# wjqkkky/TTS

Measured on AMD Instinct MI355X. Metric: mel-frames/s (Tacotron2-DDC + MB-MelGAN end-to-end), higher is better.
Workload: dtype f32; 1 GPU; C2: Tacotron2-DDC (r_init=7, r=2, sigmoid attn) + MB-MelGAN [8,4,2]x4, 32 LJ-length utterances per GPU; global_batch=32, r=2, parallelism=replicas x1

## Files before the change

tts_amd/_lib.py:

```python

import atexit
import collections
import ctypes
import os
import threading
from typing import Dict

import numpy as np

_HERE = os.path.dirname(os.path.abspath(__file__))
LIB_PATH = os.environ.get("TTSHIP_LIB", os.path.join(_HERE, "libttship.so"))

_lib = None
_lock = threading.Lock()

_c_int_p = ctypes.POINTER(ctypes.c_int32)
_c_i64_p = ctypes.POINTER(ctypes.c_int64)
_c_f_p = ctypes.POINTER(ctypes.c_float)
_c_i_p = ctypes.POINTER(ctypes.c_int)
_vp = ctypes.c_void_p

SIGNATURES = [
    ("tts_version", ctypes.c_int, []),
    ("tts_last_error", ctypes.c_char_p, []),
# ... 449 lines not shown
    def pqmf_analysis(self, x, lens, H, y):
        B, L = x.shape
        l_a, l_p = _i32(lens)
        _check(self.lib.tts_pqmf_analysis(self.h, _ptr(x), l_p, B, L, H.shape[0], _ptr(H), H.shape[1] - 1, _ptr(y),
                                          y.shape[2], _stream(x.device)))

    def stft_pair_sums(self, y_hat, y, nsamples, n_fft, win_length, hop_length, sums):
        B, L = y.shape
        n_a, n_p = _i32(nsamples)
        _check(self.lib.tts_stft_pair_sums(self.h, _ptr(y_hat), _ptr(y), n_p, B, L, int(n_fft), int(win_length),
                                           int(hop_length), _ptr(sums), _stream(y.device)))

    def torch_stft_mag(self, wav, nsamples, n_fft, win_length, hop_length, mag):
        B, L = wav.shape
        n_a, n_p = _i32(nsamples)
        _check(self.lib.tts_torch_stft_mag(self.h, _ptr(wav), n_p, B, L, int(n_fft), int(win_length),
                                           int(hop_length), _ptr(mag), mag.shape[2], _stream(wav.device)))

    def conv_test(self, weight, bias, lens, src, out, max_q, device, transposed=False, K=1, dil=1, nphase=1,
                  pad_left=(0,), merged_u=0, src2=None, resid=None, resid_rows=0, aux=None, auxb=0, len_add=0,
                  in_mul=1, q_mul=1, out_mul=1, rep_pad=0, pad_mode=0, epi=0):
        w = np.ascontiguousarray(weight, dtype=np.float32)
        b = np.ascontiguousarray(bias, dtype=np.float32)
        lens_a = np.ascontiguousarray(lens, dtype=np.int32)
        d = ConvTest()
        d.h_weight, d.h_bias, d.h_lens = w.ctypes.data, b.ctypes.data, lens_a.ctypes.data
        d.transposed = int(bool(transposed))
        if transposed:
            d.Cin, d.Cout = w.shape[0], w.shape[1]
        else:
            d.Cout, d.Cin = w.shape[-3], w.shape[-2]
        assert len(b) == d.Cout
        d.K, d.dil, d.nphase, d.merged_u = K, dil, nphase, merged_u
        for i, p in enumerate(pad_left):
            d.pad_left[i] = p
        d.nsrc = 1 if src2 is None else 2
        for i, s in enumerate((src,) if src2 is None else (src, src2)):
            d.d_src[i] = s[0]
            for j in range(3):
                d.src_strides[i][j] = s[1][j]
            d.src_C[i], d.src_act[i] = s[2], s[3]
        d.d_out = out[0]
        for j in range(3):
            d.out_strides[j] = out[1][j]
        if resid is not None:
            d.d_resid = resid[0]
            for j in range(3):
                d.resid_strides[j] = resid[1][j]
        d.resid_rows, d.d_aux, d.auxb = resid_rows, aux, auxb
        d.B, d.max_q, d.len_add, d.in_mul, d.q_mul, d.out_mul = len(lens_a), max_q, len_add, in_mul, q_mul, out_mul
        d.rep_pad, d.pad_mode, d.epi = rep_pad, pad_mode, epi
        with self.lock:
            _check(self.lib.tts_test_conv(self.h, ctypes.c_void_p(ctypes.addressof(d)), _stream(device)))
        return bool(d.ran_x3), int(d.tq), int(d.range_flag)

    def decoder_stats(self):
        path, n = ctypes.c_int(0), ctypes.c_int(0)
        ms = (ctypes.c_float * 4)()
        st = (ctypes.c_int * 4)()
        _check(self.lib.tts_decoder_stats(self.h, ctypes.byref(path), ctypes.byref(n), ms, st))
        return int(path.value), [(float(ms[i]), int(st[i])) for i in range(n.value)]

    def set_gemm_mode(self, mode: str):
        if mode not in ("x3", "f32"):
            raise ValueError("gemm mode must be 'x3' or 'f32'")
        with self.lock:
            _check(self.lib.tts_set_gemm_mode(self.h, 1 if mode == "x3" else 0))

    def gemm_mode(self):
        m, n = ctypes.c_int(0), ctypes.c_int64(0)
        _check(self.lib.tts_gemm_mode(self.h, ctypes.byref(m), ctypes.byref(n)))
        return ("x3" if m.value else "f32"), int(n.value)

    def time_decoder_kernel(self, which: int, iters: int) -> float:
        ms = ctypes.c_float(0.0)
        _check(self.lib.tts_time_decoder_kernel(self.h, which, iters, ctypes.byref(ms)))
        return float(ms.value)


_engines: Dict[int, Engine] = {}


def get_engine(device) -> Engine:
    import torch
    dev = torch.device(device)
    if dev.type != "cuda":
        raise RuntimeError("tts_amd runs on MI355X (ROCm 'cuda' devices) only; got device "
                           f"'{dev}'. There is no CPU fallback: move the model with .cuda().")
    idx = dev.index if dev.index is not None else torch.cuda.current_device()
    with _lock:
        eng = _engines.get(idx)
    if eng is None:
        eng = Engine(idx)
        with _lock:
            _engines[idx] = eng
    return eng


@atexit.register
def _close_engines():
    with _lock:
        engines = list(_engines.values())
        _engines.clear()
    for eng in engines:
        try:
            eng.close()
# ... 3 lines not shown
```

tts_amd/csrc/api_core.hip:

```cpp
#include "host.h"
#include "split16.h"
#include "switches.h"

#include <cmath>
#include <cstring>
#include <memory>

static thread_local std::string g_err;
void tts_set_error(const std::string& m) { g_err = m; }

namespace ttsh {

__global__ void put_rows_kernel(int* dst, RowInts r, int n) {
  if ((int)threadIdx.x < n) dst[threadIdx.x] = r.v[threadIdx.x];
}

const int* put_rows(int* dst, const int32_t* h, int n, hipStream_t s) {
  for (int o = 0; o < n; o += BMAX) {
    const int m = std::min(BMAX, n - o);
    put_rows_kernel<<<1, BMAX, 0, s>>>(dst + o, row_ints(h + o, m), m);
    HIP_OK(hipGetLastError());
  }
  return dst;
}
// ... 147 lines not shown
  for (float v : Wm) wm_in_range &= std::fabs(v) < F16_RANGE;
  if (wm_in_range && conv_x3_supported(Cin, u * Cout, 2, 1)) {
    std::vector<float> bm((size_t)u * Cout);
    for (size_t r = 0; r < bm.size(); ++r) bm[r] = bias[r / u];
    pack_conv_x3_only(Lm, merge_convT_phases(Wm, u, Cin, Cout), bm, Cin, u * Cout, 2);
  } else {
    Lm.W16.reset();
  }
}

ConvRan run_conv(const ConvLayer& L, const ConvCall& c, hipStream_t st) {
  ConvArgs a{};
  a.src[0] = c.s[0];
  a.src[1] = c.nsrc > 1 ? c.s[1] : c.s[0];
  if (c.nsrc == 1) a.src[0].C = L.Cin;
  a.nsrc = c.nsrc;
  a.Cin = L.Cin;
  a.K = L.K;
  a.dil = L.dil;
  a.pad_mode = c.pad_mode;
  a.lens = c.lens;
  a.len_add = c.len_add;
  a.in_mul = c.in_mul;
  a.q_mul = c.q_mul;
  a.rep_pad = c.rep_pad;
  a.nphase = L.nphase;
  for (int i = 0; i < 8; ++i) a.pad_left[i] = L.pad_left[i];
  a.w_phase_stride = L.phase_stride;
  a.W = L.W.f();
  a.bias = L.bias.f();
  a.Cout = L.Cout;
  a.Cout_pad = L.Cout_pad;
  a.out = c.out;
  a.ob = c.ob;
  a.oc = c.oc;
  a.ot = c.ot;
  a.out_mul = c.out_mul;
  a.epi_act = c.epi;
  a.resid = c.resid;
  a.rb = c.rb;
  a.rc = c.rc;
  a.rt = c.rt;
  a.resid_rows = c.resid_rows;
  a.aux = c.aux;
  a.auxb = c.auxb;
  a.max_q = c.max_q;
  a.B = c.B;
  a.merged_u = c.merged_u;
  TTS_CHECK(!c.merged_u || (c.oflow && L.W16.p), "phase-merged ConvTranspose runs on split-f16 weights only");
  if (c.oflow && L.W16.p && c.nsrc == 1 && (c.s[0].sc != 1 || c.s[0].st % 4 == 0)) {
    a.W16 = L.W16.p;
    a.w16_phase_stride = L.w16_stride;
    a.oflow = c.oflow;
    return {true, launch_conv_x3(a, st)};
  }
  return {false, launch_conv(a, L.tile, st)};
}

void enter(tts_ctx* c, void* stream, bool join_voc) {
  if (c->sv_live && join_voc) {
    HIP_OK(hipStreamWaitEvent(c->s, c->ev_sv, 0));
    c->sv_live = false;
  }
  if (hipStreamQuery((hipStream_t)stream) == hipSuccess) return;
  (void)hipGetLastError();
  HIP_OK(hipEventRecord(c->ev_in, (hipStream_t)stream));
  HIP_OK(hipStreamWaitEvent(c->s, c->ev_in, 0));
}
void leave(tts_ctx* c, void* stream) {
  HIP_OK(hipEventRecord(c->ev_out, c->s));
  HIP_OK(hipStreamWaitEvent((hipStream_t)stream, c->ev_out, 0));
}

std::vector<float> lstm_tile_rows(const std::vector<float>& W, int H, int K) {
  std::vector<float> out((size_t)4 * H * K);
  for (int t = 0; t < H / 4; ++t)
    for (int g = 0; g < 4; ++g)
      for (int u = 0; u < 4; ++u) {
        const size_t src = (size_t)(g * H + 4 * t + u) * K, dst = (size_t)(t * 16 + g * 4 + u) * K;
        std::memcpy(&out[dst], &W[src], K * sizeof(float));
      }
  return out;
}

std::vector<float> hcat(const std::vector<std::pair<const float*, int>>& parts, int rows) {
  int K = 0;
  for (auto& p : parts) K += p.second;
  std::vector<float> out((size_t)rows * K);
  for (int r = 0; r < rows; ++r) {
    int off = 0;
    for (auto& p : parts) {
      std::memcpy(&out[(size_t)r * K + off], p.first + (size_t)r * p.second, p.second * sizeof(float));
      off += p.second;
    }
  }
  return out;
}

std::vector<float> slice_cols(const std::vector<float>& W, int rows, int K, int c0, int c1) {
  std::vector<float> out((size_t)rows * (c1 - c0));
  for (int r = 0; r < rows; ++r)
    std::memcpy(&out[(size_t)r * (c1 - c0)], &W[(size_t)r * K + c0], (c1 - c0) * sizeof(float));
  return out;
}

std::vector<float> swz(const std::vector<float>& Wm, int rows, int K) {
// ... 103 lines not shown
int tts_test_conv(tts_ctx* c, tts_conv_test* d, void* stream) {
  return guarded_ctx(c, [&] {
    TTS_CHECK(d && d->h_weight && d->h_bias && d->h_lens && d->d_src[0] && d->d_out, "test_conv: null argument");
    TTS_CHECK(d->Cin >= 1 && d->Cout >= 1 && d->B >= 1 && d->max_q >= 0, "test_conv: sizes");
    TTS_CHECK(d->nsrc == 1 || (d->nsrc == 2 && d->d_src[1] && d->src_C[0] + d->src_C[1] == d->Cin), "test_conv: sources");
    TTS_CHECK(d->nphase >= 1 && d->nphase <= 8, "conv: nphase");
    auto lay = [](const int64_t* s) {
      TTS_CHECK(s[1] >= 0 && s[2] >= 0 && s[1] < (1L << 31) && s[2] < (1L << 31), "test_conv: strides");
      return Layout{(long)s[0], (int)s[1], (int)s[2]};
    };
    d->ran_x3 = d->tq = 0;
    d->range_flag = 0;
    DeviceGuard g(c->device);
    enter(c, stream);
    ConvLayer L, Lm;
    const std::vector<float> bias(d->h_bias, d->h_bias + d->Cout);
    if (d->transposed) {
      const int u = d->nphase;
      TTS_CHECK(d->merged_u == 0 || d->merged_u == u, "test_conv: merged_u is 0 or the stride");
      pack_convT(L, Lm, std::vector<float>(d->h_weight, d->h_weight + (size_t)d->Cin * d->Cout * 2 * u), bias, u,
                 d->Cin, d->Cout);
    } else {
      TTS_CHECK(d->K >= 1 && d->dil >= 1 && d->merged_u == 0, "test_conv: taps");
      const size_t n = (size_t)d->nphase * d->Cout * d->Cin * d->K;
      pack_conv(L, std::vector<float>(d->h_weight, d->h_weight + n), bias, d->Cin, d->Cout, d->K, d->dil, d->nphase,
                d->pad_left);
    }
    DevBuf lens;
    ConvCall cc = conv_call(c, put_rows(lens, d->h_lens, d->B, c->s), d->B, d->max_q);
    cc.in(d->d_src[0], lay(d->src_strides[0]), d->nsrc == 2 ? d->src_C[0] : d->Cin, d->src_act[0]);
    if (d->nsrc == 2) {
      cc.in2(d->d_src[1], lay(d->src_strides[1]), d->src_C[1]);
      cc.s[1].act = d->src_act[1];
    }
    cc.to(d->d_out, lay(d->out_strides));
    if (d->d_resid) cc.add(d->d_resid, lay(d->resid_strides));
    cc.resid_rows = d->resid_rows;
    cc.aux = d->d_aux;
    cc.auxb = (long)d->auxb;
    cc.pad_mode = d->pad_mode;
    cc.len_add = d->len_add;
    cc.in_mul = d->in_mul;
    cc.q_mul = d->q_mul;
    cc.out_mul = d->out_mul;
    cc.rep_pad = d->rep_pad;
    cc.epi = d->epi;
    cc.merged_u = d->merged_u;
    if (cc.oflow) HIP_OK(hipMemsetAsync(cc.oflow, 0, 4, c->s));
    struct Sync {
      hipStream_t s;
      ~Sync() { (void)hipStreamSynchronize(s); }
    } sync{c->s};
    const ConvRan ran = run_conv(d->merged_u ? Lm : L, cc, c->s);
    d->ran_x3 = ran.x3 ? 1 : 0;
    d->tq = ran.tq;
    if (cc.oflow) HIP_OK(hipMemcpyAsync(&c->pinned[PIN_FLAG], cc.oflow, 4, hipMemcpyDeviceToHost, c->s));
    HIP_OK(hipStreamSynchronize(c->s));
    if (cc.oflow) d->range_flag = (uint32_t)c->pinned[PIN_FLAG];
    leave(c, stream);
  });
}

int tts_gemm_mode(tts_ctx* c, int* mode, int64_t* fallbacks) {
  return guarded_ctx(c, [&] {
    TTS_CHECK(mode && fallbacks, "null argument");
    *mode = c->gemm_x3 ? 1 : 0;
    *fallbacks = c->x3_fallbacks;
  });
}

}
```

tts_amd/csrc/common.h:

```cpp
#pragma once
#include <hip/hip_runtime.h>
#include <atomic>
#include <cstdint>
#include <mutex>
#include <set>
#include <string>
#include <tuple>
#include <vector>

typedef float f32x4 __attribute__((ext_vector_type(4)));

constexpr int BMAX = 64;

struct RowInts {
  int v[BMAX];
};

#define MFMA16(a, b, c) __builtin_amdgcn_mfma_f32_16x16x4f32((a), (b), (c), 0, 0, 0)

void tts_set_error(const std::string& msg);

#define HIP_OK(expr)                                                                   \
  do {                                                                                 \
    hipError_t _e = (expr);                                                            \
// ... 51 lines not shown
  return __builtin_copysignf((1.f - e) * __builtin_amdgcn_rcpf(1.f + e), x);
}

struct ConvSrc {
  const float* ptr;
  long sb;
  int sc, st;
  int C;
  int act;
};

struct ConvArgs {
  ConvSrc src[2];
  int nsrc;
  int Cin;
  int K, dil;
  int pad_mode;
  const int* lens;
  int len_add;
  int in_mul;
  int q_mul;
  int rep_pad;
  int nphase;
  int pad_left[8];
  long w_phase_stride;
  const float* W;
  const float* bias;
  int Cout, Cout_pad;
  float* out;
  long ob;
  int oc, ot;
  int out_mul;
  int epi_act;
  const float* resid;
  long rb;
  int rc, rt;
  int resid_rows;
  const float* aux;
  long auxb;
  int max_q;
  int B;
  const void* W16 = nullptr;
  long w16_phase_stride = 0;
  unsigned* oflow = nullptr;
  int merged_u = 0;
};

enum ConvTile { TILE_128x64 = 0, TILE_64x64, TILE_192x64, TILE_96x64, TILE_48x128, TILE_80x64, TILE_16x256 };
int conv_tile_tc(int tile);
int conv_tile_for_cout(int cout);
int launch_conv(const ConvArgs& a, int tile, hipStream_t s);
bool conv_x3_supported(int Cin, int Cout, int K, int dil);
int launch_conv_x3(const ConvArgs& a, hipStream_t s);
std::vector<uint16_t> pack_conv_x3(const std::vector<float>& Wm, int Cin, int Cout, int K, int nphase,
                                   long* phase_stride_bytes);
std::vector<float> merge_convT_phases(const std::vector<float>& Wm, int u, int Cin, int Cout);

void swizzle_rows16(const float* Wm, int rows, int rows_pad, int Kdim, float* dst);

struct FillList {
  static constexpr int N = 32;
  int n = 0;
  void* p[N];
  long words[N];
  unsigned val[N];
  void add(void* ptr, size_t bytes, unsigned v = 0) {
    TTS_CHECK(n < N && bytes % 4 == 0, "FillList: too many entries or unaligned size");
    if (!bytes) return;
    p[n] = ptr;
    words[n] = (long)(bytes / 4);
    val[n] = v;
    ++n;
  }
};
void launch_fills(const FillList& f, hipStream_t s);

void launch_pqmf_synthesis(const float* x, long xb, long xc, const float* G, int N, int taps,
                           const int* lens, int len_add, int L_mul, int maxL, int B, float* y, long yb,
                           hipStream_t s);

struct ResArgs {
  const float* x;
  float* y;
  long sb;
  int Ls;
  const int* lens;
  int len_add, mul;
  int dil;
  const float* Wd;
  const float* bd;
  const float* Wf;
  const float* bf;
  int max_q, B;
  const void* Wd16 = nullptr;
  const void* Wf16 = nullptr;
  unsigned* oflow = nullptr;
};
void launch_resblock(const ResArgs& a, int C, hipStream_t s);
bool resblock_x3_supported(int C);
void launch_resblock_x3(const ResArgs& a, const int* h_lens, int C, hipStream_t s);
void pack_resblock_x3(const std::vector<float>& wd, const std::vector<float>& wf, int C,
                      std::vector<uint16_t>& wd16, std::vector<uint16_t>& wf16);
void pack_resblock_x3p(const std::vector<float>& wd, int C, std::vector<uint16_t>& wd16);

struct StackArgs {
  const float* x;
// ... 30 lines not shown
```

tts_amd/csrc/conv_epi.h:

```cpp
#pragma once
#include "common.h"

constexpr int CONV_MAX_SPAN = 7;

__device__ __forceinline__ int map_pad_index(int i, int L, int mode, bool& valid) {
  if (i >= 0 && i < L) return i;
  if (mode == 0) {
    valid = false;
    return 0;
  }
  if (mode == 1) {
    if (i < 0) i = -i;
    if (i >= L) i = 2 * (L - 1) - i;
  }
  return i < 0 ? 0 : (i >= L ? L - 1 : i);
}

template <int MI, int NI, int WN>
__device__ __forceinline__ void conv_epilogue(const ConvArgs& a, f32x4 (&acc)[MI][NI], int b, int ph, int q0,
                                              int co0, int wm, int wn, int lane) {
  const int base = a.lens[b] + a.len_add;
  const int Lq = base * a.q_mul;
  const int qb = wn * 16 * NI + (lane & 15);
  const int g4 = 4 * (lane >> 4);
#pragma unroll
  for (int mi = 0; mi < MI; ++mi) {
    float bias4[4];
#pragma unroll
    for (int j = 0; j < 4; ++j) {
      const int co = min(co0 + wm * 16 * MI + mi * 16 + g4 + j, a.Cout - 1);
      bias4[j] = a.bias[co];
    }
#pragma unroll
    for (int ni = 0; ni < NI; ++ni) {
      const int q = q0 + qb + ni * 16;
      if (q >= Lq) continue;
      const int t = q * a.out_mul + ph;
      if (a.epi_act == 5) {
        const int co = co0 + wm * 16 * MI + mi * 16 + g4;
        if (co >= a.Cout) continue;
        const int m2 = co >> 1, Ch = a.Cout >> 1;
        const float* xs = a.resid + (long)b * a.rb + (long)t * a.rt;
        float in[4];
        in[0] = xs[(long)m2 * a.rc];
        in[1] = xs[(long)(m2 + 1) * a.rc];
#pragma unroll
        for (int p = 0; p < 2; ++p) {
          const float u = acc[mi][ni][2 * p] + bias4[2 * p], g = acc[mi][ni][2 * p + 1] + bias4[2 * p + 1];
          in[2 + p] = (xs[(long)(Ch + m2 + p) * a.rc] - u) * expf(-g);
        }
        float* os = a.out + (long)b * a.ob + (long)t * a.ot;
#pragma unroll
        for (int o = 0; o < 4; ++o) {
          const int c = (o < 2 ? 0 : Ch) + m2 + (o & 1);
          const float* w = a.aux + c * 6;
          float v = w[0] * in[0];
          v = fmaf(w[1], in[1], v);
          v = fmaf(w[2], in[2], v);
          v = fmaf(w[3], in[3], v);
          os[(long)c * a.oc] = (v - w[4]) * w[5];
        }
        continue;
      }
      if (a.epi_act >= 3) {
#pragma unroll
        for (int j = 0; j < 4; j += 2) {
          const int co = co0 + wm * 16 * MI + mi * 16 + g4 + j;
          if (co >= a.Cout) continue;
// ... 29 lines not shown
```

tts_amd/csrc/conv_x3.hip:

```cpp
#include "common.h"
#include "conv_epi.h"
#include "split16.h"
#include "switches.h"
#include "x3_tile.h"

#include <algorithm>
#include <mutex>
#include <map>

namespace {
constexpr int CX_XR = 80;
}

template <int MI, int NI, int WM, int WN, int KT, int RS, int SD>
__global__ __launch_bounds__(64 * WM * WN) void conv_x3_kernel(ConvArgs a, int nq, int nco, int nz) {
  constexpr int NTHR = 64 * WM * WN;
  constexpr int TC = 16 * MI * WM, TQ = 16 * NI * WN;
  constexpr int SPT = (4 * (TQ + CONV_MAX_SPAN) + NTHR - 1) / NTHR;
  static_assert(RS == KT || RS == 2 * KT, "weight ring: one or two chunks of taps");
  extern __shared__ __attribute__((aligned(16))) _Float16 shx[];

  const int ntile = nq * nco * nz;
  const int per = (ntile + 7) / 8;
  const int w = (int)(blockIdx.x % 8) * per + (int)(blockIdx.x / 8);
// ... 118 lines not shown
  stage_store(X0, st[0], 0);
  if constexpr (SD == 2) {
    if (NCH > 1) stage_load(st[1], 1);
    if (NCH > 2) stage_load(st[0], 2);
  }
  lds_barrier();
  for (int ch0 = 0; ch0 < NCH; ch0 += 2) {
#pragma unroll
    for (int p = 0; p < 2; ++p) {
      const int ch = ch0 + p;
      if (ch < NCH) {
        const _Float16* X = p ? X1 : X0;
        if constexpr (SD == 1) {
          if (ch + 1 < NCH) stage_load(st[0], ch + 1);
          __builtin_amdgcn_sched_barrier(0);
        }
#pragma unroll
        for (int kq = 0; kq < KT; ++kq) {
          constexpr bool TWO = RS == 2 * KT;
          const int slot = TWO ? p * KT + kq : kq;
          h8 bh[NI], bl[NI];
#pragma unroll
          for (int ni = 0; ni < NI; ++ni) {
            const _Float16* q = X + (nb + ni * 16 + kq * dil) * CX_XR + kg;
            bh[ni] = *reinterpret_cast<const h8*>(q);
            bl[ni] = *reinterpret_cast<const h8*>(q + 32);
          }
          __builtin_amdgcn_sched_barrier(0);
#pragma unroll
          for (int mi = 0; mi < MI; ++mi)
#pragma unroll
            for (int ni = 0; ni < NI; ++ni)
              mfma_x3(ring[slot][mi][0], ring[slot][mi][1], bh[ni], bl[ni], am[mi][ni], ac[mi][ni]);
          wload(ring[slot], ch * KT + kq + RS);
          __builtin_amdgcn_sched_barrier(0);
        }
        if constexpr (SD == 2) {
          if (ch + 1 < NCH) stage_store(p ? X0 : X1, st[p ^ 1], ch + 1);
          if (ch + 3 < NCH) stage_load(st[p ^ 1], ch + 3);
        } else {
          if (ch + 1 < NCH) stage_store(p ? X0 : X1, st[0], ch + 1);
        }
        lds_barrier();
      }
    }
  }
  f32x4 acc[MI][NI];
#pragma unroll
  for (int mi = 0; mi < MI; ++mi)
#pragma unroll
    for (int ni = 0; ni < NI; ++ni)
#pragma unroll
      for (int j = 0; j < 4; ++j) acc[mi][ni][j] = x3_value(am[mi][ni][j], ac[mi][ni][j]);
  const bool vec = a.merged_u && a.ot == 1 && (a.oc & 3) == 0 && (a.ob & 3) == 0 &&
                   (reinterpret_cast<uintptr_t>(a.out) & 15) == 0 && a.Cout % 16 == 0;
  if (vec && a.merged_u % 4 == 0) {
    const int u = a.merged_u, L = Lin;
    float* ob = a.out + (long)b * a.ob;
#pragma unroll
    for (int mi = 0; mi < MI; ++mi) {
      const int m0 = co0 + wm * 16 * MI + mi * 16 + 4 * (lane >> 4);
      if (m0 >= a.Cout) continue;
      const int co = m0 / u, phs0 = m0 - co * u;
      const int hi0 = 2 * phs0 >= u, hi1 = 2 * (phs0 + 2) >= u;
      const f32x4 bias{a.bias[m0], a.bias[m0 + 1], a.bias[m0 + 2], a.bias[m0 + 3]};
      float* orow = ob + (long)co * a.oc;
#pragma unroll
      for (int ni = 0; ni < NI; ++ni) {
        const int q = q0 + nb + ni * 16;
        const f32x4 v = acc[mi][ni] + bias;
        if (u % 8 == 0) {
          if (q - hi0 >= 0 && q - hi0 < L) *reinterpret_cast<f32x4*>(orow + (long)(q - hi0) * u + phs0) = v;
        } else {
          typedef float f2 __attribute__((ext_vector_type(2)));
          if (q - hi0 >= 0 && q - hi0 < L) *reinterpret_cast<f2*>(orow + (long)(q - hi0) * u + phs0) = f2{v[0], v[1]};
          if (q - hi1 >= 0 && q - hi1 < L) *reinterpret_cast<f2*>(orow + (long)(q - hi1) * u + phs0 + 2) = f2{v[2], v[3]};
        }
      }
    }
  } else if (vec && a.merged_u == 2) {
    typedef float f2 __attribute__((ext_vector_type(2)));
    const int L = Lin;
    float* ob = a.out + (long)b * a.ob;
    const int r = lane & 15;
#pragma unroll
    for (int mi = 0; mi < MI; ++mi) {
      const int m0 = co0 + wm * 16 * MI + mi * 16 + 4 * (lane >> 4);
      if (m0 >= a.Cout) continue;
#pragma unroll
      for (int c = 0; c < 2; ++c) {
        const int co = m0 / 2 + c;
        const float b0 = a.bias[m0 + 2 * c], b1 = a.bias[m0 + 2 * c + 1];
        float* orow = ob + (long)co * a.oc;
#pragma unroll
        for (int ni = 0; ni < NI; ++ni) {
          const float v0 = acc[mi][ni][2 * c] + b0;
          const float v1 = acc[mi][ni][2 * c + 1] + b1;
          const float down = __shfl_down(v1, 1, 16);
          const float wrap = ni + 1 < NI ? __shfl(acc[mi][ni + 1 < NI ? ni + 1 : ni][2 * c + 1] + b1, lane & ~15) : 0.f;
          const int q = q0 + nb + ni * 16;
          const bool last = r == 15 && ni == NI - 1;
          if (q >= 0 && q < L) {
            if (last) orow[2 * q] = v0;
            else *reinterpret_cast<f2*>(orow + 2 * q) = f2{v0, r < 15 ? down : wrap};
          }
          if (r == 0 && ni == 0 && q - 1 >= 0 && q - 1 < L) orow[2 * q - 1] = v1;
        }
      }
    }
  } else if (a.merged_u) {
    const int u = a.merged_u, L = Lin;
    float* ob = a.out + (long)b * a.ob;
#pragma unroll
    for (int mi = 0; mi < MI; ++mi)
#pragma unroll
      for (int j = 0; j < 4; ++j) {
        const int m = co0 + wm * 16 * MI + mi * 16 + 4 * (lane >> 4) + j;
        if (m >= a.Cout) continue;
        const int co = m / u, phs = m - co * u;
        const int hi = 2 * phs >= u;
        const float bias = a.bias[m];
#pragma unroll
        for (int ni = 0; ni < NI; ++ni) {
          const int qq = q0 + nb + ni * 16 - hi;
#ifdef CX_PROBE_NOSTORE
          if (qq >= 0 && qq < L && acc[mi][ni][j] + bias == 12345.f) ob[(long)co * a.oc + (long)(qq * u + phs) * a.ot] = 0.f;
#else
          if (qq >= 0 && qq < L) ob[(long)co * a.oc + (long)(qq * u + phs) * a.ot] = acc[mi][ni][j] + bias;
#endif
        }
      }
  } else {
    conv_epilogue<MI, NI, WN>(a, acc, b, ph, q0, co0, wm, wn, lane);
  }
  if (bad) __hip_atomic_fetch_or(a.oflow, 1u, __ATOMIC_RELAXED, __HIP_MEMORY_SCOPE_AGENT);
}

enum { CX_T128 = 0, CX_T192, CX_T96, CX_T64, CX_T80, CX_T48, CX_NONE };

static int cx_tile(int Cout) {
  if (Cout % 128 == 0) return CX_T128;
  if (Cout == 192) return CX_T192;
  if (Cout == 96) return CX_T96;
  if (Cout == 80) return CX_T80;
  if (Cout == 48) return CX_T48;
  if (Cout % 64 == 0) return CX_T64;
  if (Cout % 80 == 0) return CX_T80;
  return CX_NONE;
}

bool conv_x3_supported(int Cin, int Cout, int K, int dil) {
  return Cin % 8 == 0 && Cin >= 8 && cx_tile(Cout) != CX_NONE && (K == 1 || K == 2 || K == 3 || K == 5 || K == 7) &&
         (K - 1) * dil <= CONV_MAX_SPAN;
}

template <int MI, int NI, int WM, int WN, int KT, int RS, int SD>
static int cx_launch(const ConvArgs& a, hipStream_t s) {
  constexpr int TC = 16 * MI * WM, TQ = 16 * NI * WN;
  ensure_dyn_lds((const void*)conv_x3_kernel<MI, NI, WM, WN, KT, RS, SD>, 160 * 1024);
  const int nq = (a.max_q + TQ - 1) / TQ, nco = (a.Cout + TC - 1) / TC, nz = a.B * a.nphase;
  const long ntile = (long)nq * nco * nz;
  TTS_CHECK(ntile < (1L << 30), "conv_x3: grid too large");
  const int per = (int)((ntile + 7) / 8);
  const size_t lds = (size_t)2 * (TQ + (KT - 1) * a.dil) * CX_XR * 2;
  conv_x3_kernel<MI, NI, WM, WN, KT, RS, SD><<<dim3(8 * per), 64 * WM * WN, lds, s>>>(a, nq, nco, nz);
  return TQ;
}

template <int MI, int NI, int WM, int WN, int KT, int RS, int SD>
static long cx_cost_k(const ConvArgs& a) {
  constexpr int TC = 16 * MI * WM, TQ = 16 * NI * WN;
  const void* f = (const void*)conv_x3_kernel<MI, NI, WM, WN, KT, RS, SD>;
  const size_t lds = (size_t)2 * (TQ + (KT - 1) * a.dil) * CX_XR * 2;
  static std::mutex mu;
  static std::map<size_t, long> slots_by_lds;
  long slots;
  ensure_dyn_lds(f, 160 * 1024);
  const int cus = device_cu_count();
  {
    std::lock_guard<std::mutex> lk(mu);
    auto it = slots_by_lds.find(lds);
    if (it == slots_by_lds.end()) {
      int nb = 0;
      HIP_OK(hipOccupancyMaxActiveBlocksPerMultiprocessor(&nb, f, 64 * WM * WN, lds));
// ... 89 lines not shown
```

tts_amd/csrc/host.h:

```cpp
#pragma once
#include "common.h"
#include "launch.h"
#include "../../include/ttship.h"

#include <algorithm>
#include <functional>
#include <map>
#include <mutex>
#include <stdexcept>
#include <string>
#include <vector>

struct DecCtlBlock;
struct DecDev;

namespace ttsh {

constexpr int CHUNK = 8;

struct DevBuf {
  void* p = nullptr;
  size_t bytes = 0;
  DevBuf() = default;
  DevBuf(const DevBuf&) = delete;
// ... 54 lines not shown
struct HostMapConsumer {
  HostMap& m;
  ~HostMapConsumer() { m.clear(); }
};

struct ConvLayer {
  DevBuf W, bias;
  int Cin = 0, Cout = 0, Cout_pad = 0, K = 1, dil = 1, tile = 0, nphase = 1;
  int pad_left[8] = {0};
  long phase_stride = 0;
  DevBuf W16;
  long w16_stride = 0;
};

void pack_conv(ConvLayer& L, const std::vector<float>& Wm, const std::vector<float>& bias, int Cin, int Cout,
               int K, int dil, int nphase, const int* pad_left);
void pack_conv_x3_only(ConvLayer& L, const std::vector<float>& Wm, const std::vector<float>& bias, int Cin, int Cout,
                       int K);

struct Layout {
  long b;
  int c, t;
};
inline Layout bct(int C, long T) { return {(long)C * T, (int)T, 1}; }
inline Layout btc(long T, int C) { return {T * C, 1, C}; }

struct ConvCall {
  ConvCall& in(const float* p, Layout l, int C, int act = 0) { return s[0] = ConvSrc{p, l.b, l.c, l.t, C, act}, *this; }
  ConvCall& in2(const float* p, Layout l, int C) { return s[1] = ConvSrc{p, l.b, l.c, l.t, C, 0}, nsrc = 2, *this; }
  ConvCall& to(float* p, Layout l) { return out = p, ob = l.b, oc = l.c, ot = l.t, *this; }
  ConvCall& add(const float* p, Layout l) { return resid = p, rb = l.b, rc = l.c, rt = l.t, *this; }
  ConvSrc s[2];
  int nsrc = 1;
  int pad_mode = 0;
  const int* lens = nullptr;
  int len_add = 0, in_mul = 1, q_mul = 1, rep_pad = 0, out_mul = 1;
  float* out = nullptr;
  long ob = 0;
  int oc = 0, ot = 0;
  int epi = 0;
  const float* resid = nullptr;
  long rb = 0;
  int rc = 0, rt = 0, resid_rows = 0;
  const float* aux = nullptr;
  long auxb = 0;
  int max_q = 0, B = 0;
  unsigned* oflow = nullptr;
  int merged_u = 0;
};

struct ConvRan {
  bool x3 = false;
  int tq = 0;
};
ConvRan run_conv(const ConvLayer& L, const ConvCall& c, hipStream_t st);

void pack_convT(ConvLayer& L, ConvLayer& Lm, const std::vector<float>& wt, const std::vector<float>& bias, int u,
                int Cin, int Cout);

std::vector<float> lstm_tile_rows(const std::vector<float>& W, int H, int K);
std::vector<float> hcat(const std::vector<std::pair<const float*, int>>& parts, int rows);
std::vector<float> slice_cols(const std::vector<float>& W, int rows, int K, int c0, int c1);
std::vector<float> swz(const std::vector<float>& Wm, int rows, int K);
void fold_convbn(const HostMap& m, const std::string& pfx, int Cin, int Cout, int K, std::vector<float>& Wm,
                 std::vector<float>& bias);

struct TacoModel {
  bool ready = false;
  int num_chars = 0, r_init = 7, softmax = 0;
  DevBuf emb;
  ConvLayer enc[3], lstm_in, penc, post[5];
  DevBuf whhT;
  DevBuf whhT16;
  DevBuf pre1, pre2, att_p, att_pre, att_bias, dec_w, dec_bias, WqT, Wloc, Wdense, v, proj_w, proj_b;
  DevBuf att_p_x3, dec_x3, apre_x3, pj_x3;
  DevBuf Wcomb;
  float bv = 0.f;
  std::vector<float> proj_rows, proj_bias, pre1_host;
  DevBuf pj_w, pj_b;
  int pj_r = -1;
  int spk_dim = 0, num_spk = 0;
  bool prenet_bn = false, windowing = false, forward_attn = false, trans_agent = false, forward_attn_mask = false;
  std::vector<float> pre1_bias;
  DevBuf pre1_b0, pre2_b, ta_w;
  float ta_b = 0.f;
  bool variant() const { return prenet_bn || windowing || forward_attn || graves; }
  bool graves = false;
  int graves_K = 0;
  DevBuf na1_w, na1_b, na2_w, na2_b;
  DevBuf spk_table;
  std::vector<float> spk_att_h, spk_dec_h, spk_penc_h, proj_spk;
  DevBuf spk_wT;
  int gst_dim = 0, gst_heads = 0, gst_ntok = 0, gst_es_q = 0, es = 0;
  DevBuf gst_cw[6], gst_cb[6];
  DevBuf gst_wihT, gst_whhT, gst_bih, gst_bhh, gst_wqT, gst_K, gst_V;
};

struct GstWS {
  DevBuf a, b;
};

constexpr int PMAX_LAUNCH = 4;
constexpr int PBAR_CAND = 16;
constexpr int ENC_NDOM_MAX = 4;
constexpr int TS_ENC = 16, TS_DEC = TS_ENC + ENC_NDOM_MAX, TS_RES = TS_DEC + PMAX_LAUNCH, TS_FLAG = TS_RES + 3 * BMAX,
              TS_END = TS_FLAG + 1, TS_VERR = TS_END + PMAX_LAUNCH, TS_N = TS_VERR + 1;
// ... 394 lines not shown
```

tts_amd/csrc/switches.h:

```cpp
#pragma once
#include <cstdlib>
#include <string>

namespace sw {

inline bool on_unless_zero(const char* name, bool dflt) {
  const char* e = std::getenv(name);
  return e ? std::atoi(e) != 0 : dflt;
}
inline bool on_unless_one(const char* name) {
  const char* e = std::getenv(name);
  return !e || std::atoi(e) != 1;
}
inline bool present(const char* name) { return std::getenv(name) != nullptr; }
inline int number(const char* name, int dflt) {
  const char* e = std::getenv(name);
  return e ? std::atoi(e) : dflt;
}
inline std::string text(const char* name) {
  const char* e = std::getenv(name);
  return e ? e : "";
}

inline bool gemm_f32() { static const bool v = text("TTS_GEMM") == "f32"; return v; }
inline bool voc_stream() { static const bool v = on_unless_zero("TTS_VOC_STREAM", true); return v; }

inline double barrier_timeout_ms() {
  static const double v = [] {
    const char* e = std::getenv("TTS_BARRIER_TIMEOUT_MS");
    const double ms = e ? std::atof(e) : 2000.0;
    return ms < 1.0 ? 1.0 : (ms > 40000.0 ? 40000.0 : ms);
  }();
  return v;
}
inline bool coop_launch() { static const bool v = on_unless_zero("TTS_COOP_LAUNCH", false); return v; }
inline bool bar_calibrate() { static const bool v = on_unless_zero("TTS_BAR_CALIBRATE", true); return v; }
inline bool diag_xcc() { static const bool v = present("TTS_DIAG_XCC"); return v; }

inline bool encoder_steps() { static const bool v = text("TTS_ENCODER") == "steps"; return v; }
inline bool lstm_row_groups() { static const bool v = on_unless_one("TTS_LSTM_RG"); return v; }
inline bool decoder_graph() { static const bool v = text("TTS_DECODER") == "graph"; return v; }
inline bool decoder_f32() { static const bool v = present("TTS_DECODER_F32"); return v; }
inline bool align_in_p4() { static const bool v = present("TTS_ALIGN_IN_P4"); return v; }
inline const char* ptrace_file() {
  static const bool set = present("TTS_PTRACE");
  static const std::string v = text("TTS_PTRACE");
  return set ? v.c_str() : nullptr;
}
inline int ptrace_t0() { static const int v = number("TTS_PTRACE_T0", 100); return v; }
inline int ptrace_launch() { static const int v = number("TTS_PTRACE_LAUNCH", 0); return v; }

inline bool stack_fuse() { static const bool v = on_unless_zero("TTS_STACK_FUSE", true); return v; }
inline bool stack_fuse96() { static const bool v = on_unless_zero("TTS_STACK_FUSE96", false); return v; }
inline bool ct_fuse() { static const bool v = on_unless_zero("TTS_CT_FUSE", true); return v; }
inline int cx_ni128() { static const int v = number("TTS_CX_NI128", 0); return v; }

inline bool ge2e_pipe() { static const bool v = text("TTS_GE2E_PIPE") != "0"; return v; }

inline int pwgan_staging() {
  static const int v = [] {
    const std::string e = text("TTS_PWGAN_STAGING");
    return e == "regs" ? 0 : e == "ring4" ? 2 : 1;
  }();
  return v;
}
inline int pwgan_tile() { static const int v = number("TTS_PWGAN_TILE", 0); return v; }

}
```

Before: 1.340 million mel-frames/s.

## Add persistent wide-tile kernel for phase-merged ConvTranspose upsampling

Adds a persistent kernel for phase-merged ConvTranspose layers with K=2. Each block is 12 waves wide and covers 384 output rows per tile. It double-buffers split-f16 input staging in LDS, prefetches weights in a register ring, and loops over tiles spread across XCD-aligned block groups. The goal is more reuse of each staged input tile across output channels and less launch and tail overhead than the generic x3 conv path. The merged-store epilogue moves into a shared helper, and the new path is on by default behind TTS_CONVT_WIDE. The risks are higher register and LDS pressure, and lower occupancy on small layers.

```diff
diff --git a/tts_amd/_lib.py b/tts_amd/_lib.py
--- a/tts_amd/_lib.py
+++ b/tts_amd/_lib.py
@@ -525,6 +525,7 @@
         d.rep_pad, d.pad_mode, d.epi = rep_pad, pad_mode, epi
         with self.lock:
             _check(self.lib.tts_test_conv(self.h, ctypes.c_void_p(ctypes.addressof(d)), _stream(device)))
+        self.conv_test_kernel = int(d.ran_x3)
         return bool(d.ran_x3), int(d.tq), int(d.range_flag)
 
     def decoder_stats(self):
diff --git a/tts_amd/csrc/api_core.hip b/tts_amd/csrc/api_core.hip
--- a/tts_amd/csrc/api_core.hip
+++ b/tts_amd/csrc/api_core.hip
@@ -223,6 +223,7 @@
     a.W16 = L.W16.p;
     a.w16_phase_stride = L.w16_stride;
     a.oflow = c.oflow;
+    if (sw::convt_wide() && convt_wide_fits(a)) return {true, launch_convt_wide(a, st), true};
     return {true, launch_conv_x3(a, st)};
   }
   return {false, launch_conv(a, L.tile, st)};
@@ -432,7 +433,7 @@
       ~Sync() { (void)hipStreamSynchronize(s); }
     } sync{c->s};
     const ConvRan ran = run_conv(d->merged_u ? Lm : L, cc, c->s);
-    d->ran_x3 = ran.x3 ? 1 : 0;
+    d->ran_x3 = ran.wide ? 2 : ran.x3 ? 1 : 0;
     d->tq = ran.tq;
     if (cc.oflow) HIP_OK(hipMemcpyAsync(&c->pinned[PIN_FLAG], cc.oflow, 4, hipMemcpyDeviceToHost, c->s));
     HIP_OK(hipStreamSynchronize(c->s));
diff --git a/tts_amd/csrc/common.h b/tts_amd/csrc/common.h
--- a/tts_amd/csrc/common.h
+++ b/tts_amd/csrc/common.h
@@ -127,6 +127,8 @@
 int launch_conv(const ConvArgs& a, int tile, hipStream_t s);
 bool conv_x3_supported(int Cin, int Cout, int K, int dil);
 int launch_conv_x3(const ConvArgs& a, hipStream_t s);
+bool convt_wide_fits(const ConvArgs& a);
+int launch_convt_wide(const ConvArgs& a, hipStream_t s);
 std::vector<uint16_t> pack_conv_x3(const std::vector<float>& Wm, int Cin, int Cout, int K, int nphase,
                                    long* phase_stride_bytes);
 std::vector<float> merge_convT_phases(const std::vector<float>& Wm, int u, int Cin, int Cout);
diff --git a/tts_amd/csrc/conv_epi.h b/tts_amd/csrc/conv_epi.h
--- a/tts_amd/csrc/conv_epi.h
+++ b/tts_amd/csrc/conv_epi.h
@@ -14,6 +14,86 @@
     if (i >= L) i = 2 * (L - 1) - i;
   }
   return i < 0 ? 0 : (i >= L ? L - 1 : i);
+}
+
+template <int MI, int NI>
+__device__ __forceinline__ void convt_merged_store(const ConvArgs& a, const f32x4 (&acc)[MI][NI],
+                                                   const float (&bias4)[MI][4], int b, int qw, int mw, int lane, int L) {
+  const int u = a.merged_u;
+  const bool vec = a.ot == 1 && (a.oc & 3) == 0 && (a.ob & 3) == 0 && (reinterpret_cast<uintptr_t>(a.out) & 15) == 0 &&
+                   a.Cout % 16 == 0;
+  float* ob = a.out + (long)b * a.ob;
+  if (vec && u % 4 == 0) {
+#pragma unroll
+    for (int mi = 0; mi < MI; ++mi) {
+      const int m0 = mw + mi * 16 + 4 * (lane >> 4);
+      if (m0 >= a.Cout) continue;
+      const int co = m0 / u, phs0 = m0 - co * u;
+      const int hi0 = 2 * phs0 >= u, hi1 = 2 * (phs0 + 2) >= u;
+      const f32x4 bias{bias4[mi][0], bias4[mi][1], bias4[mi][2], bias4[mi][3]};
+      float* orow = ob + (long)co * a.oc;
+#pragma unroll
+      for (int ni = 0; ni < NI; ++ni) {
+        const int q = qw + ni * 16;
+        const f32x4 v = acc[mi][ni] + bias;
+        if (u % 8 == 0) {
+          if (q - hi0 >= 0 && q - hi0 < L) *reinterpret_cast<f32x4*>(orow + (long)(q - hi0) * u + phs0) = v;
+        } else {
+          typedef float f2 __attribute__((ext_vector_type(2)));
+          if (q - hi0 >= 0 && q - hi0 < L) *reinterpret_cast<f2*>(orow + (long)(q - hi0) * u + phs0) = f2{v[0], v[1]};
+          if (q - hi1 >= 0 && q - hi1 < L) *reinterpret_cast<f2*>(orow + (long)(q - hi1) * u + phs0 + 2) = f2{v[2], v[3]};
+        }
+      }
+    }
+  } else if (vec && u == 2) {
+    typedef float f2 __attribute__((ext_vector_type(2)));
+    const int r = lane & 15;
+#pragma unroll
+    for (int mi = 0; mi < MI; ++mi) {
+      const int m0 = mw + mi * 16 + 4 * (lane >> 4);
+      if (m0 >= a.Cout) continue;
+#pragma unroll
+      for (int c = 0; c < 2; ++c) {
+        const int co = m0 / 2 + c;
+        const float b0 = bias4[mi][2 * c], b1 = bias4[mi][2 * c + 1];
+        float* orow = ob + (long)co * a.oc;
+#pragma unroll
+        for (int ni = 0; ni < NI; ++ni) {
+          const float v0 = acc[mi][ni][2 * c] + b0;
+          const float v1 = acc[mi][ni][2 * c + 1] + b1;
+          const float down = __shfl_down(v1, 1, 16);
+          const float wrap = ni + 1 < NI ? __shfl(acc[mi][ni + 1 < NI ? ni + 1 : ni][2 * c + 1] + b1, lane & ~15) : 0.f;
+          const int q = qw + ni * 16;
+          const bool last = r == 15 && ni == NI - 1;
+          if (q >= 0 && q < L) {
+            if (last) orow[2 * q] = v0;
+            else *reinterpret_cast<f2*>(orow + 2 * q) = f2{v0, r < 15 ? down : wrap};
+          }
+          if (r == 0 && ni == 0 && q - 1 >= 0 && q - 1 < L) orow[2 * q - 1] = v1;
+        }
+      }
+    }
+  } else {
+#pragma unroll
+    for (int mi = 0; mi < MI; ++mi)
+#pragma unroll
+      for (int j = 0; j < 4; ++j) {
+        const int m = mw + mi * 16 + 4 * (lane >> 4) + j;
+        if (m >= a.Cout) continue;
+        const int co = m / u, phs = m - co * u;
+        const int hi = 2 * phs >= u;
+        const float bias = bias4[mi][j];
+#pragma unroll
+        for (int ni = 0; ni < NI; ++ni) {
+          const int qq = qw + ni * 16 - hi;
+#ifdef CX_PROBE_NOSTORE
+          if (qq >= 0 && qq < L && acc[mi][ni][j] + bias == 12345.f) ob[(long)co * a.oc + (long)(qq * u + phs) * a.ot] = 0.f;
+#else
+          if (qq >= 0 && qq < L) ob[(long)co * a.oc + (long)(qq * u + phs) * a.ot] = acc[mi][ni][j] + bias;
+#endif
+        }
+      }
+  }
 }
 
 template <int MI, int NI, int WN>
diff --git a/tts_amd/csrc/conv_x3.hip b/tts_amd/csrc/conv_x3.hip
--- a/tts_amd/csrc/conv_x3.hip
+++ b/tts_amd/csrc/conv_x3.hip
@@ -194,84 +194,13 @@
     for (int ni = 0; ni < NI; ++ni)
 #pragma unroll
       for (int j = 0; j < 4; ++j) acc[mi][ni][j] = x3_value(am[mi][ni][j], ac[mi][ni][j]);
-  const bool vec = a.merged_u && a.ot == 1 && (a.oc & 3) == 0 && (a.ob & 3) == 0 &&
-                   (reinterpret_cast<uintptr_t>(a.out) & 15) == 0 && a.Cout % 16 == 0;
-  if (vec && a.merged_u % 4 == 0) {
-    const int u = a.merged_u, L = Lin;
-    float* ob = a.out + (long)b * a.ob;
-#pragma unroll
-    for (int mi = 0; mi < MI; ++mi) {
-      const int m0 = co0 + wm * 16 * MI + mi * 16 + 4 * (lane >> 4);
-      if (m0 >= a.Cout) continue;
-      const int co = m0 / u, phs0 = m0 - co * u;
-      const int hi0 = 2 * phs0 >= u, hi1 = 2 * (phs0 + 2) >= u;
-      const f32x4 bias{a.bias[m0], a.bias[m0 + 1], a.bias[m0 + 2], a.bias[m0 + 3]};
-      float* orow = ob + (long)co * a.oc;
-#pragma unroll
-      for (int ni = 0; ni < NI; ++ni) {
-        const int q = q0 + nb + ni * 16;
-        const f32x4 v = acc[mi][ni] + bias;
-        if (u % 8 == 0) {
-          if (q - hi0 >= 0 && q - hi0 < L) *reinterpret_cast<f32x4*>(orow + (long)(q - hi0) * u + phs0) = v;
-        } else {
-          typedef float f2 __attribute__((ext_vector_type(2)));
-          if (q - hi0 >= 0 && q - hi0 < L) *reinterpret_cast<f2*>(orow + (long)(q - hi0) * u + phs0) = f2{v[0], v[1]};
-          if (q - hi1 >= 0 && q - hi1 < L) *reinterpret_cast<f2*>(orow + (long)(q - hi1) * u + phs0 + 2) = f2{v[2], v[3]};
-        }
-      }
-    }
-  } else if (vec && a.merged_u == 2) {
-    typedef float f2 __attribute__((ext_vector_type(2)));
-    const int L = Lin;
-    float* ob = a.out + (long)b * a.ob;
-    const int r = lane & 15;
-#pragma unroll
-    for (int mi = 0; mi < MI; ++mi) {
-      const int m0 = co0 + wm * 16 * MI + mi * 16 + 4 * (lane >> 4);
-      if (m0 >= a.Cout) continue;
-#pragma unroll
-      for (int c = 0; c < 2; ++c) {
-        const int co = m0 / 2 + c;
-        const float b0 = a.bias[m0 + 2 * c], b1 = a.bias[m0 + 2 * c + 1];
-        float* orow = ob + (long)co * a.oc;
-#pragma unroll
-        for (int ni = 0; ni < NI; ++ni) {
-          const float v0 = acc[mi][ni][2 * c] + b0;
-          const float v1 = acc[mi][ni][2 * c + 1] + b1;
-          const float down = __shfl_down(v1, 1, 16);
-          const float wrap = ni + 1 < NI ? __shfl(acc[mi][ni + 1 < NI ? ni + 1 : ni][2 * c + 1] + b1, lane & ~15) : 0.f;
-          const int q = q0 + nb + ni * 16;
-          const bool last = r == 15 && ni == NI - 1;
-          if (q >= 0 && q < L) {
-            if (last) orow[2 * q] = v0;
-            else *reinterpret_cast<f2*>(orow + 2 * q) = f2{v0, r < 15 ? down : wrap};
-          }
-          if (r == 0 && ni == 0 && q - 1 >= 0 && q - 1 < L) orow[2 * q - 1] = v1;
-        }
-      }
-    }
-  } else if (a.merged_u) {
-    const int u = a.merged_u, L = Lin;
-    float* ob = a.out + (long)b * a.ob;
+  if (a.merged_u) {
+    float bias4[MI][4];
 #pragma unroll
     for (int mi = 0; mi < MI; ++mi)
 #pragma unroll
-      for (int j = 0; j < 4; ++j) {
-        const int m = co0 + wm * 16 * MI + mi * 16 + 4 * (lane >> 4) + j;
-        if (m >= a.Cout) continue;
-        const int co = m / u, phs = m - co * u;
-        const int hi = 2 * phs >= u;
-        const float bias = a.bias[m];
-#pragma unroll
-        for (int ni = 0; ni < NI; ++ni) {
-          const int qq = q0 + nb + ni * 16 - hi;
-#ifdef CX_PROBE_NOSTORE
-          if (qq >= 0 && qq < L && acc[mi][ni][j] + bias == 12345.f) ob[(long)co * a.oc + (long)(qq * u + phs) * a.ot] = 0.f;
-#else
-          if (qq >= 0 && qq < L) ob[(long)co * a.oc + (long)(qq * u + phs) * a.ot] = acc[mi][ni][j] + bias;
-#endif
-        }
-      }
+      for (int j = 0; j < 4; ++j) bias4[mi][j] = a.bias[min(co0 + wm * 16 * MI + mi * 16 + 4 * (lane >> 4) + j, a.Cout - 1)];
+    convt_merged_store<MI, NI>(a, acc, bias4, b, q0 + nb, co0 + wm * 16 * MI, lane, Lin);
   } else {
     conv_epilogue<MI, NI, WN>(a, acc, b, ph, q0, co0, wm, wn, lane);
   }
diff --git a/tts_amd/csrc/convt_wide.hip b/tts_amd/csrc/convt_wide.hip
--- /dev/null
+++ b/tts_amd/csrc/convt_wide.hip
@@ -0,0 +1,246 @@
+#include "common.h"
+#include "conv_epi.h"
+#include "split16.h"
+#include "x3_tile.h"
+
+#include <algorithm>
+#include <type_traits>
+
+namespace {
+constexpr int CW_XR = 80;
+constexpr int CW_MI = 2;
+constexpr int CW_WAVES = 12;
+constexpr int CW_ROWS = 16 * CW_MI * CW_WAVES;
+constexpr int CW_MAXM = 4096;
+}
+
+template <int WAVES, int MI, int NI, int NB>
+__global__ __launch_bounds__(64 * WAVES) void convt_wide_kernel(ConvArgs a, int ngroups) {
+  constexpr int NTHR = 64 * WAVES;
+  constexpr int TQ = 16 * NI;
+  constexpr int ROWS = TQ + 1;
+  constexpr int SPT = (8 * ROWS + NTHR - 1) / NTHR;
+  static_assert(NI % NB == 0, "B operands in groups of NB n-tiles");
+  __shared__ __attribute__((aligned(16))) _Float16 xs[2][ROWS * CW_XR];
+  __shared__ __attribute__((aligned(16))) float sbias[CW_MAXM];
+  __shared__ int tcum[65], tlen[64];
+
+  const int tid = threadIdx.x;
+  const int lane = tid & 63, wave = __builtin_amdgcn_readfirstlane(tid >> 6);
+  const int nb = lane & 15;
+  const int kg = 8 * (lane >> 4);
+  const int kgx[2] = {kg ^ lds_rsw(nb), kg ^ lds_rsw(nb + 1)};
+  const int NCH = a.Cin / 32;
+  const int NKS = 2 * NCH;
+  const int mtiles = a.Cout / 16;
+  const ConvSrc& S = a.src[0];
+  bool bad = false;
+
+  if (wave == 0) {
+    const int L = lane < a.B ? (a.lens[lane] + a.len_add) * a.q_mul : 0;
+    x3_tile_scan<TQ>(tcum, tlen, lane, L > 0 ? L + 1 : 0);
+  }
+  for (int i = tid; i < a.Cout; i += NTHR) sbias[i] = a.bias[i];
+  __syncthreads();
+  const int npt = __builtin_amdgcn_readfirstlane(tcum[64]);
+  const int ntile = npt * ngroups;
+  const int per = (ntile + 7) / 8, wpx = (int)gridDim.x / 8;
+  const int xbase = (int)(blockIdx.x % 8) * per;
+  const int xend = min(xbase + per, ntile);
+  int w = xbase + (int)(blockIdx.x / 8);
+  if (w >= xend) return;
+
+  int sg[SPT], srow[SPT];
+  bool sitem[SPT];
+#pragma unroll
+  for (int j = 0; j < SPT; ++j) {
+    const int e = tid + NTHR * j;
+    sg[j] = min(e / ROWS, 7), srow[j] = e % ROWS, sitem[j] = e < 8 * ROWS;
+  }
+  struct Tile {
+    __amdgpu_buffer_rsrc_t xr;
+    int b, q0, L, mt0;
+    int voff[SPT];
+    bool sval[SPT];
+  };
+  auto tile_at = [&](int i) {
+    const int g = i / npt;
+    const X3Tile t = x3_tile_of<TQ>(tcum, tlen, a.B, lane, i - g * npt);
+    Tile T;
+    T.b = t.b, T.q0 = t.q0, T.L = t.L - 1, T.mt0 = g * (MI * WAVES);
+    T.xr = __builtin_amdgcn_make_buffer_rsrc(
+        const_cast<float*>(S.ptr + (long)T.b * S.sb), 0,
+        (int)min((long)0x7fffffff, ((long)(S.C - 1) * S.sc + (long)(T.L - 1) * S.st + 1) * 4), 0x00020000);
+#pragma unroll
+    for (int j = 0; j < SPT; ++j) {
+      const int pos = T.q0 - 1 + srow[j];
+      T.sval[j] = sitem[j] && pos >= 0 && pos < T.L;
+      T.voff[j] = sitem[j] ? (sg[j] * 4 * S.sc + min(max(pos, 0), T.L - 1) * S.st) * 4 : 0x7fffffff;
+    }
+    return T;
+  };
+  const int act = S.act;
+  float st[2][SPT][4];
+  auto stage_load2 = [&](const Tile& T0, const Tile& T1, bool second, float (&sr)[SPT][4], int ch) {
+    const int cb = 32 * ch * S.sc * 4;
+    const __amdgpu_buffer_rsrc_t xr = second ? T1.xr : T0.xr;
+#pragma unroll
+    for (int j = 0; j < SPT; ++j) {
+      const int voff = second ? T1.voff[j] : T0.voff[j];
+#pragma unroll
+      for (int c = 0; c < 4; ++c)
+        sr[j][c] = __uint_as_float(__builtin_amdgcn_raw_buffer_load_b32(xr, voff, cb + c * S.sc * 4, 0));
+    }
+  };
+  auto stage_load = [&](const Tile& T, float (&sr)[SPT][4], int ch) { stage_load2(T, T, false, sr, ch); };
+  auto stage_store = [&](_Float16* X, const Tile& T, const float (&sr)[SPT][4]) {
+#pragma unroll
+    for (int j = 0; j < SPT; ++j) {
+      if (sitem[j]) {
+        float mx = 0.f;
+        f32x4 v;
+#pragma unroll
+        for (int c = 0; c < 4; ++c) {
+          v[c] = T.sval[j] ? sr[j][c] : 0.f;
+          mx = __builtin_elementwise_maximum(mx, __builtin_fabsf(v[c]));
+          if (act) v[c] = lrelu02(v[c]);
+        }
+        bad |= !(mx < F16_RANGE);
+        h4 hi, lo;
+        split4(v, hi, lo);
+        const int sx = (4 * sg[j]) ^ lds_rsw(srow[j]);
+        *reinterpret_cast<h4*>(X + srow[j] * CW_XR + sx) = hi;
+        *reinterpret_cast<h4*>(X + srow[j] * CW_XR + 32 + sx) = lo;
+      }
+    }
+  };
+
+  const __amdgpu_buffer_rsrc_t wr = x3_rsrc(a.W16);
+  const int wlo = lane * 32;
+  h8 ring[2][MI][2];
+  auto wload = [&](h8 (&r)[MI][2], int mtb, int ks) {
+#pragma unroll
+    for (int mi = 0; mi < MI; ++mi) {
+      const int mt = min(mtb + wave * MI + mi, mtiles - 1);
+      x3_load_a(r[mi], wr, wlo, (mt * NKS + ks) * 2048);
+    }
+  };
+
+  f32x4 am[MI][NI], ac[MI][NI];
+  Tile cur = tile_at(w), nxt = cur;
+  auto chunk = [&](auto PC, int ch, bool even) {
+    constexpr int P = decltype(PC)::value;
+    const _Float16* X = xs[P];
+    const bool wrap = ch + 1 >= NCH;
+#pragma unroll
+    for (int kq = 0; kq < 2; ++kq) {
+#pragma unroll
+      for (int n0 = 0; n0 < NI; n0 += NB) {
+        h8 bh[NB], bl[NB];
+#pragma unroll
+        for (int nj = 0; nj < NB; ++nj) {
+          const _Float16* q = X + (nb + (n0 + nj) * 16 + kq) * CW_XR + kgx[kq];
+          bh[nj] = *reinterpret_cast<const h8*>(q);
+          bl[nj] = *reinterpret_cast<const h8*>(q + 32);
+        }
+        __builtin_amdgcn_sched_barrier(0);
+#pragma unroll
+        for (int mi = 0; mi < MI; ++mi)
+#pragma unroll
+          for (int nj = 0; nj < NB; ++nj)
+            mfma_x3(ring[kq][mi][0], ring[kq][mi][1], bh[nj], bl[nj], am[mi][n0 + nj], ac[mi][n0 + nj]);
+      }
+      wload(ring[kq], wrap ? nxt.mt0 : cur.mt0, wrap ? kq : 2 * (ch + 1) + kq);
+      __builtin_amdgcn_sched_barrier(0);
+    }
+    if (ch + 1 < NCH) stage_store(xs[P ^ 1], cur, st[P ^ 1]);
+    else if (even) stage_store(xs[P ^ 1], nxt, st[P ^ 1]);
+    const bool over = ch + 3 >= NCH;
+    stage_load2(cur, nxt, over, st[P ^ 1], min(over ? ch + 3 - NCH : ch + 3, NCH - 1));
+    lds_barrier();
+  };
+  using P0 = std::integral_constant<int, 0>;
+  using P1 = std::integral_constant<int, 1>;
+
+  stage_load(cur, st[0], 0);
+#pragma unroll
+  for (int kq = 0; kq < 2; ++kq) wload(ring[kq], cur.mt0, kq);
+  stage_load(cur, st[1], min(1, NCH - 1));
+  stage_store(xs[0], cur, st[0]);
+  stage_load(cur, st[0], min(2, NCH - 1));
+  lds_barrier();
+  for (;;) {
+    const int wn = w + wpx;
+    const bool more = wn < xend;
+    if (more) nxt = tile_at(wn);
+    else nxt = cur;
+    if (NCH == 2) stage_load(nxt, st[0], 0);
+#pragma unroll
+    for (int mi = 0; mi < MI; ++mi)
+#pragma unroll
+      for (int ni = 0; ni < NI; ++ni) am[mi][ni] = ac[mi][ni] = f32x4{0.f, 0.f, 0.f, 0.f};
+    int ch = 0;
+    for (; ch + 1 < NCH; ch += 2) {
+      chunk(P0{}, ch, true);
+      chunk(P1{}, ch + 1, true);
+    }
+    if (ch < NCH) {
+      chunk(P0{}, ch, false);
+      stage_load(nxt, st[0], 0);
+      stage_load(nxt, st[1], min(1, NCH - 1));
+    }
+    f32x4 acc[MI][NI];
+#pragma unroll
+    for (int mi = 0; mi < MI; ++mi)
+#pragma unroll
+      for (int ni = 0; ni < NI; ++ni)
+#pragma unroll
+        for (int j = 0; j < 4; ++j) acc[mi][ni][j] = x3_value(am[mi][ni][j], ac[mi][ni][j]);
+    float bias4[MI][4];
+#pragma unroll
+    for (int mi = 0; mi < MI; ++mi) {
+      const f32x4 bv = *reinterpret_cast<const f32x4*>(sbias + min((cur.mt0 + wave * MI + mi) * 16 + 4 * (lane >> 4), a.Cout - 4));
+#pragma unroll
+      for (int j = 0; j < 4; ++j) bias4[mi][j] = bv[j];
+    }
+    convt_merged_store<MI, NI>(a, acc, bias4, cur.b, cur.q0 + nb, (cur.mt0 + wave * MI) * 16, lane, cur.L);
+    if (!more) break;
+    if (NCH & 1) {
+      stage_store(xs[0], nxt, st[0]);
+      stage_load(nxt, st[0], min(2, NCH - 1));
+      lds_barrier();
+    }
+    cur = nxt;
+    w = wn;
+  }
+  if (bad) __hip_atomic_fetch_or(a.oflow, 1u, __ATOMIC_RELAXED, __HIP_MEMORY_SCOPE_AGENT);
+}
+
+bool convt_wide_fits(const ConvArgs& a) {
+  const int last = a.Cout % CW_ROWS;
+  return a.merged_u > 0 && a.W16 && a.oflow && a.nsrc == 1 && a.K == 2 && a.dil == 1 && a.nphase == 1 &&
+         a.Cout % 16 == 0 && (last == 0 || 2 * last >= CW_ROWS) && a.Cin % 32 == 0 && a.Cin >= 32 && a.B <= 64 && a.Cout <= CW_MAXM &&
+         a.in_mul == a.q_mul;
+}
+
+template <int WAVES, int MI, int NI, int NB>
+static int cw_launch(const ConvArgs& a, hipStream_t s) {
+  constexpr int TQ = 16 * NI, GROUP = 16 * MI * WAVES;
+  const int ngroups = (a.Cout + GROUP - 1) / GROUP;
+  const long bound = (long)((a.max_q + TQ - 1) / TQ) * a.B * ngroups;
+  TTS_CHECK(bound < (1L << 30), "convt_wide: too many tiles");
+  const int wpx = (int)std::max<long>(1, std::min<long>(device_cu_count() / 8, (bound + 7) / 8));
+  convt_wide_kernel<WAVES, MI, NI, NB><<<dim3(8 * wpx), 64 * WAVES, 0, s>>>(a, ngroups);
+  return TQ;
+}
+
+int launch_convt_wide(const ConvArgs& a, hipStream_t s) {
+  TTS_CHECK(convt_wide_fits(a), "convt_wide: unsupported call");
+  TTS_CHECK(a.src[0].C == a.Cin && a.pad_left[0] == 1 && a.pad_mode == 0 && a.epi_act == 0 && a.rep_pad == 0 &&
+                a.Cout % a.merged_u == 0 && a.merged_u % 2 == 0,
+            "convt_wide: phase-merged ConvTranspose arguments");
+  if (a.max_q <= 0 || a.B <= 0) return 0;
+  const int tq = cw_launch<CW_WAVES, CW_MI, 4, 1>(a, s);
+  HIP_OK(hipGetLastError());
+  return tq;
+}
diff --git a/tts_amd/csrc/host.h b/tts_amd/csrc/host.h
--- a/tts_amd/csrc/host.h
+++ b/tts_amd/csrc/host.h
@@ -130,6 +130,7 @@
 struct ConvRan {
   bool x3 = false;
   int tq = 0;
+  bool wide = false;
 };
 ConvRan run_conv(const ConvLayer& L, const ConvCall& c, hipStream_t st);
 
diff --git a/tts_amd/csrc/switches.h b/tts_amd/csrc/switches.h
--- a/tts_amd/csrc/switches.h
+++ b/tts_amd/csrc/switches.h
@@ -54,6 +54,7 @@
 inline bool stack_fuse96() { static const bool v = on_unless_zero("TTS_STACK_FUSE96", false); return v; }
 inline bool ct_fuse() { static const bool v = on_unless_zero("TTS_CT_FUSE", true); return v; }
 inline int cx_ni128() { static const int v = number("TTS_CX_NI128", 0); return v; }
+inline bool convt_wide() { static const bool v = on_unless_zero("TTS_CONVT_WIDE", true); return v; }
 
 inline bool ge2e_pipe() { static const bool v = text("TTS_GE2E_PIPE") != "0"; return v; }
 
```

New measurement: 1.333 million mel-frames/s. No clear change (-0.5%).
